# knagrecha/saturn

Measured on AMD Instinct MI355X. Metric: samples_per_s, higher is better.
Workload: dtype bf16; 1 GPU; model=gptj-6b, global_batch=16, seq_len=512, parallelism=dp1, optimizer=fused_sgd

## Files before the change

saturn_amd/ops/csrc/attention.hip:

```cpp

#include <torch/extension.h>
#include <ATen/hip/HIPContext.h>

#include <atomic>

#include "common.h"
#include "ops.h"

namespace samd {

typedef __attribute__((ext_vector_type(8))) short bf16x8;
typedef __attribute__((ext_vector_type(4))) float f32x4;

constexpr int QBLK = 64;
constexpr int KBLK = 32;
constexpr int WROWS = 16;

struct TStr {
  long sb, sh, st;
};
static TStr str_of(const at::Tensor& t) {
  return TStr{t.stride(0), t.stride(1), t.stride(2)};
}

// ... 130 lines not shown
#pragma unroll
      for (int c = 0; c < CHUNKS; ++c) {
        const int idx = (c * 256 + threadIdx.x) * 8;
        const int row = idx / D, col = idx % D;
        stg_k[c] = *reinterpret_cast<const bf16x8*>(
            Kh + (long)(kv0 + KBLK + row) * ks.st + col);
        stg_v[c] = *reinterpret_cast<const bf16x8*>(
            Vh + (long)(kv0 + KBLK + row) * vs.st + col);
      }
    }
    __syncthreads();

    f32x4 acc0 = {0.f, 0.f, 0.f, 0.f};
    f32x4 acc1 = {0.f, 0.f, 0.f, 0.f};
#pragma unroll
    for (int ds = 0; ds < D / 32; ++ds) {
      bf16x8 bk0 = *reinterpret_cast<const bf16x8*>(&lds.k[r][ds * 32 + qg * 8]);
      bf16x8 bk1 =
          *reinterpret_cast<const bf16x8*>(&lds.k[16 + r][ds * 32 + qg * 8]);
      acc0 = __builtin_amdgcn_mfma_f32_16x16x32_bf16(frag_q[ds], bk0, acc0, 0, 0, 0);
      acc1 = __builtin_amdgcn_mfma_f32_16x16x32_bf16(frag_q[ds], bk1, acc1, 0, 0, 0);
    }
#pragma unroll
    for (int reg = 0; reg < 4; ++reg) {
      const int row = qg * 4 + reg;
      const int qrow = q0 + row;
      float s0 = acc0[reg] * scale;
      float s1 = acc1[reg] * scale;
      if (causal) {
        if (kv0 + r > qrow) s0 = -INFINITY;
        if (kv0 + 16 + r > qrow) s1 = -INFINITY;
      }
      if (kv0 + r >= kv_len) s0 = -INFINITY;
      if (kv0 + 16 + r >= kv_len) s1 = -INFINITY;
      if constexpr (LO) {
        if (kv0 + r < lo_r[reg]) s0 = -INFINITY;
        if (kv0 + 16 + r < lo_r[reg]) s1 = -INFINITY;
      }
      float tm = fmaxf(s0, s1);
#pragma unroll
      for (int off = 1; off < 16; off <<= 1)
        tm = fmaxf(tm, __shfl_xor(tm, off, 64));
      const float m_new = fmaxf(m_reg[reg], tm);
      const float al =
          (m_reg[reg] == -INFINITY) ? 0.f : __expf(m_reg[reg] - m_new);
      const float p0 = (s0 == -INFINITY) ? 0.f : __expf(s0 - m_new);
      const float p1 = (s1 == -INFINITY) ? 0.f : __expf(s1 - m_new);
      float ps = p0 + p1;
#pragma unroll
      for (int off = 1; off < 16; off <<= 1)
        ps += __shfl_xor(ps, off, 64);
      l_reg[reg] = l_reg[reg] * al + ps;
      m_reg[reg] = m_new;
      lds.p[wid][row][r] = f2us(p0);
      lds.p[wid][row][16 + r] = f2us(p1);
#pragma unroll
      for (int dt = 0; dt < D / 16; ++dt) otile[dt][reg] *= al;
    }

    bf16x8 frag_p = *reinterpret_cast<const bf16x8*>(&lds.p[wid][r][qg * 8]);
#pragma unroll
    for (int dt = 0; dt < D / 16; ++dt) {
      bf16x8 bv = tr16_bfrag<D + 8>(&lds.v[qg * 8][dt * 16], lane);
      otile[dt] = __builtin_amdgcn_mfma_f32_16x16x32_bf16(frag_p, bv, otile[dt], 0, 0, 0);
    }
  }

  unsigned short* Oh = O + b * os.sb + h * os.sh;
#pragma unroll
  for (int reg = 0; reg < 4; ++reg) {
    int row = qg * 4 + reg;
    float linv = 1.f / l_reg[reg];
#pragma unroll
    for (int dt = 0; dt < D / 16; ++dt)
      Oh[(long)(q0 + row) * os.st + dt * 16 + r] =
          f2us(otile[dt][reg] * linv);
  }
  if (r == 0 && LSE != nullptr) {
#pragma unroll
    for (int reg = 0; reg < 4; ++reg)
      LSE[bh * (long)T + q0 + qg * 4 + reg] =
          m_reg[reg] + __logf(l_reg[reg]);
  }
}



typedef __attribute__((ext_vector_type(16))) float f32x16;

template <int D>
struct AttnV2Lds {
  unsigned short k[KBLK][D + 8];
  unsigned short v[KBLK][D + 8];
};

template <int D, bool LO>
__launch_bounds__(256, 2)
__global__ void attn_fwd_v2_kernel(const unsigned short* __restrict__ Q,
                                   const unsigned short* __restrict__ K,
                                   const unsigned short* __restrict__ V,
                                   unsigned short* __restrict__ O,
                                   float* __restrict__ LSE, int T,
                                   int n_heads, int n_kv, float scale,
                                   int causal, int kv_len, TStr qs,
                                   TStr ks, TStr vs,
                                   TStr os, const int* __restrict__ KVLO,
                                   long lo_sb) {
  extern __shared__ __attribute__((aligned(16))) char smem[];
  AttnV2Lds<D>& lds = *reinterpret_cast<AttnV2Lds<D>*>(smem);

  const int lane = threadIdx.x & 63;
  const int wid = threadIdx.x >> 6;
  const int qr = lane & 31;
  const int hi = lane >> 5;
  const long bh = blockIdx.x;
  const long b = bh / n_heads, h = bh % n_heads;
  const long h_kv = h * n_kv / n_heads;
  const int q0_block = blockIdx.y * (4 * 32);
  const int q0 = q0_block + wid * 32;
  const unsigned short* Qh = Q + b * qs.sb + h * qs.sh;
  const unsigned short* Kh = K + b * ks.sb + h_kv * ks.sh;
  const unsigned short* Vh = V + b * vs.sb + h_kv * vs.sh;

  constexpr bool QREG = (D < 256);
  bf16x8 frag_q[QREG ? D / 16 : 1];
  if constexpr (QREG) {
#pragma unroll
    for (int ds = 0; ds < D / 16; ++ds)
      frag_q[ds] = *reinterpret_cast<const bf16x8*>(
          Qh + (long)(q0 + qr) * qs.st + ds * 16 + hi * 8);
  }

  f32x16 oacc[D / 32];
#pragma unroll
  for (int dv = 0; dv < D / 32; ++dv)
#pragma unroll
    for (int e = 0; e < 16; ++e) oacc[dv][e] = 0.f;

  float m_row = -INFINITY, l_row = 0.f;

  int kv_begin = 0, lo_row = 0;
  if constexpr (LO) {
    const int* lo_b = KVLO + b * lo_sb;
    kv_begin = (lo_b[q0_block] / KBLK) * KBLK;
    lo_row = lo_b[q0 + qr];
  }

  constexpr int CHUNKS = (KBLK * D) / (256 * 8);
  bf16x8 stg_k[CHUNKS], stg_v[CHUNKS];
#pragma unroll
  for (int c = 0; c < CHUNKS; ++c) {
    const int idx = (c * 256 + threadIdx.x) * 8;
    const int row = idx / D, col = idx % D;
    stg_k[c] = *reinterpret_cast<const bf16x8*>(
        Kh + (long)(kv_begin + row) * ks.st + col);
    stg_v[c] = *reinterpret_cast<const bf16x8*>(
        Vh + (long)(kv_begin + row) * vs.st + col);
  }

  const int kv_end = causal ? (q0_block + 4 * 32) : T;
  for (int kv0 = kv_begin; kv0 < kv_end; kv0 += KBLK) {
    __syncthreads();
#pragma unroll
    for (int c = 0; c < CHUNKS; ++c) {
      const int idx = (c * 256 + threadIdx.x) * 8;
      const int row = idx / D, col = idx % D;
      *reinterpret_cast<bf16x8*>(&lds.k[row][col]) = stg_k[c];
      *reinterpret_cast<bf16x8*>(&lds.v[row][col]) = stg_v[c];
    }
    if (kv0 + KBLK < kv_end) {
#pragma unroll
      for (int c = 0; c < CHUNKS; ++c) {
        const int idx = (c * 256 + threadIdx.x) * 8;
        const int row = idx / D, col = idx % D;
        stg_k[c] = *reinterpret_cast<const bf16x8*>(
            Kh + (long)(kv0 + KBLK + row) * ks.st + col);
        stg_v[c] = *reinterpret_cast<const bf16x8*>(
            Vh + (long)(kv0 + KBLK + row) * vs.st + col);
      }
    }
    __syncthreads();

    f32x16 st;
#pragma unroll
    for (int e = 0; e < 16; ++e) st[e] = 0.f;
#pragma unroll
    for (int ds = 0; ds < D / 16; ++ds) {
      bf16x8 ak = *reinterpret_cast<const bf16x8*>(
          &lds.k[qr][ds * 16 + hi * 8]);
      bf16x8 fq;
      if constexpr (QREG)
        fq = frag_q[ds];
      else
        fq = *reinterpret_cast<const bf16x8*>(
            Qh + (long)(q0 + qr) * qs.st + ds * 16 + hi * 8);
      st = __builtin_amdgcn_mfma_f32_32x32x16_bf16(ak, fq, st, 0, 0, 0);
    }

    const int q_glob = q0 + qr;
    float p[16];
    float tile_max = -INFINITY;
#pragma unroll
    for (int reg = 0; reg < 16; ++reg) {
      const int key_loc = (reg & 3) + 8 * (reg >> 2) + 4 * hi;
      float sv = st[reg] * scale;
      if ((causal && kv0 + key_loc > q_glob) || kv0 + key_loc >= kv_len)
        sv = -INFINITY;
      if constexpr (LO) {
        if (kv0 + key_loc < lo_row) sv = -INFINITY;
      }
      p[reg] = sv;
      tile_max = fmaxf(tile_max, sv);
    }
    tile_max = fmaxf(tile_max, __shfl_xor(tile_max, 32, 64));
    const float m_new = fmaxf(m_row, tile_max);
    const float alpha = (m_row == -INFINITY) ? 0.f : __expf(m_row - m_new);
    float psum = 0.f;
#pragma unroll
    for (int reg = 0; reg < 16; ++reg) {
      const float pv = (p[reg] == -INFINITY) ? 0.f : __expf(p[reg] - m_new);
      p[reg] = pv;
      psum += pv;
    }
    psum += __shfl_xor(psum, 32, 64);
    l_row = l_row * alpha + psum;
    m_row = m_new;

    unsigned pk[8];
#pragma unroll
    for (int i = 0; i < 8; ++i) {
      const unsigned lo = f2us(p[2 * i]);
      const unsigned hi2 = f2us(p[2 * i + 1]);
      pk[i] = lo | (hi2 << 16);
    }
    bf16x8 pa[2];
#pragma unroll
    for (int g = 0; g < 2; ++g) {
      auto r0 = __builtin_amdgcn_permlane32_swap(pk[4 * g + 0], pk[4 * g + 2],
                                                 false, false);
      auto r1 = __builtin_amdgcn_permlane32_swap(pk[4 * g + 1], pk[4 * g + 3],
                                                 false, false);
      unsigned w0 = r0[0], w1 = r1[0], w2 = r0[1], w3 = r1[1];
      pa[g][0] = (short)(w0 & 0xffff);
      pa[g][1] = (short)(w0 >> 16);
      pa[g][2] = (short)(w1 & 0xffff);
      pa[g][3] = (short)(w1 >> 16);
      pa[g][4] = (short)(w2 & 0xffff);
      pa[g][5] = (short)(w2 >> 16);
      pa[g][6] = (short)(w3 & 0xffff);
      pa[g][7] = (short)(w3 >> 16);
    }

#pragma unroll
    for (int reg = 0; reg < 16; ++reg) {
      const int row = (reg & 3) + 8 * (reg >> 2) + 4 * hi;
      const float al = __shfl(alpha, row, 64);
#pragma unroll
      for (int dv = 0; dv < D / 32; ++dv) oacc[dv][reg] *= al;
    }

#pragma unroll
    for (int dv = 0; dv < D / 32; ++dv) {
#pragma unroll
      for (int g = 0; g < 2; ++g) {
        const int src_row = g * 16 + ((lane >> 4) & 2) * 4 + ((lane >> 2) & 3);
        const int src_col = dv * 32 + ((lane >> 4) & 1) * 16 + 4 * (lane & 3);
        const unsigned a0 = lds_addr32(&lds.v[src_row][src_col]);
        const unsigned a1 = a0 + 4u * (D + 8) * 2u;
        bf16x4 v0, v1;
        asm volatile(
            "ds_read_b64_tr_b16 %0, %2\n\t"
            "ds_read_b64_tr_b16 %1, %3\n\t"
            "s_waitcnt lgkmcnt(0)"
            : "=&v"(v0), "=&v"(v1)
            : "v"(a0), "v"(a1)
            : "memory");
        bf16x8 bv = __builtin_shufflevector(v0, v1, 0, 1, 2, 3, 4, 5, 6, 7);
        oacc[dv] = __builtin_amdgcn_mfma_f32_32x32x16_bf16(pa[g], bv,
                                                           oacc[dv], 0, 0, 0);
      }
    }
  }

  unsigned short* Oh = O + b * os.sb + h * os.sh;
  const float linv_own = 1.f / l_row;
#pragma unroll
  for (int reg = 0; reg < 16; ++reg) {
    const int row = (reg & 3) + 8 * (reg >> 2) + 4 * hi;
    const float linv = __shfl(linv_own, row, 64);
#pragma unroll
    for (int dv = 0; dv < D / 32; ++dv)
      Oh[(long)(q0 + row) * os.st + dv * 32 + qr] = f2us(oacc[dv][reg] * linv);
  }
  if (hi == 0 && LSE != nullptr)
    LSE[bh * (long)T + q0 + qr] = m_row + __logf(l_row);
}


namespace bwd {
constexpr int KB = 64;
constexpr int QT = 32;
}

template <int D, bool HASV>
struct AttnBwdLds {
  unsigned short kt[bwd::KB][D + 8];
  unsigned short vt[HASV ? bwd::KB : 1][D + 8];
  unsigned short qt[bwd::QT][D + 8];
  unsigned short dot[bwd::QT][D + 8];
  unsigned short pt[4][16][bwd::QT + 8];
  unsigned short dst[bwd::KB][bwd::QT + 8];
  float lse_t[bwd::QT];
  float delta_t[bwd::QT];
};
template <int D, bool HASV>
struct AttnBwdLdsLo : AttnBwdLds<D, HASV> {
  int lo_t[bwd::QT];
};
template <int D, bool HASV, bool LO>
using AttnBwdLdsT = typename std::conditional<LO, AttnBwdLdsLo<D, HASV>,
                                              AttnBwdLds<D, HASV>>::type;


template <int D>
__global__ void attn_delta_kernel(const unsigned short* __restrict__ dO,
                                  const unsigned short* __restrict__ O,
                                  float* __restrict__ delta, int T,
                                  int n_heads, TStr dos, TStr os) {
  const int lane = threadIdx.x & 63;
  const int wid = threadIdx.x >> 6;
  const long bh = blockIdx.y;
  const long b = bh / n_heads, h = bh % n_heads;
  const unsigned short* dOh = dO + b * dos.sb + h * dos.sh;
  const unsigned short* Oh = O + b * os.sb + h * os.sh;
  constexpr int EPL = D / 64;
  for (int t = blockIdx.x * 4 + wid; t < T; t += gridDim.x * 4) {
    float acc = 0.f;
    if constexpr (EPL >= 4) {
#pragma unroll
      for (int c = 0; c < EPL / 4; ++c) {
        const int off = (lane * (EPL / 4) + c * 64) * 4;
        bf16x4 a = *reinterpret_cast<const bf16x4*>(dOh + (long)t * dos.st + off);
        bf16x4 o4 = *reinterpret_cast<const bf16x4*>(Oh + (long)t * os.st + off);
#pragma unroll
        for (int e = 0; e < 4; ++e)
          acc += us2f((unsigned short)a[e]) * us2f((unsigned short)o4[e]);
      }
    } else {
#pragma unroll
      for (int e = 0; e < EPL; ++e) {
        const int off = lane * EPL + e;
        acc += us2f(dOh[(long)t * dos.st + off]) *
               us2f(Oh[(long)t * os.st + off]);
      }
    }
    acc = wave_allsum(acc);
    if (lane == 0) delta[bh * (long)T + t] = acc;
  }
}

template <int D, bool TR16, bool VL2, bool LO>
__launch_bounds__(256, 2)
__global__ void attn_bwd_kernel(const unsigned short* __restrict__ dO,
                                const unsigned short* __restrict__ Q,
                                const unsigned short* __restrict__ K,
                                const unsigned short* __restrict__ V,
                                const float* __restrict__ LSE,
                                const float* __restrict__ DELTA,
                                unsigned short* __restrict__ dK,
                                unsigned short* __restrict__ dV,
                                float* __restrict__ dKf,
                                float* __restrict__ dVf, int T, int n_heads,
                                int n_kv, float scale, int causal,
                                int kv_len, TStr dos,
                                TStr qs, TStr ks, TStr vs,
                                TStr dks, TStr dvs,
                                const int* __restrict__ KVLO, long lo_sb) {
  using namespace bwd;
  extern __shared__ __attribute__((aligned(16))) char smem[];
  constexpr bool HASV = (D <= 128) && !VL2;
  AttnBwdLdsT<D, HASV, LO>& lds =
      *reinterpret_cast<AttnBwdLdsT<D, HASV, LO>*>(smem);

  const int lane = threadIdx.x & 63;
  const int wid = threadIdx.x >> 6;
  const int r = lane & 15;
  const int qg = lane >> 4;
  const int kv0 = blockIdx.y * KB;
  const long bh = blockIdx.x;
  const long b = bh / n_heads, h = bh % n_heads;
  const long h_kv = h * n_kv / n_heads;
  const unsigned short* Qh = Q + b * qs.sb + h * qs.sh;
  const unsigned short* Kh = K + b * ks.sb + h_kv * ks.sh;
  const unsigned short* Vh = V + b * vs.sb + h_kv * vs.sh;
  const unsigned short* dOh = dO + b * dos.sb + h * dos.sh;
  const float* lse_h = LSE + bh * (long)T;
  const float* del_h = DELTA + bh * (long)T;
  const int* lo_b = nullptr;
  if constexpr (LO) lo_b = KVLO + b * lo_sb;

  {
    constexpr int CHUNKS = (KB * D) / (256 * 8);
#pragma unroll
    for (int c = 0; c < CHUNKS; ++c) {
      int idx = (c * 256 + threadIdx.x) * 8;
      int row = idx / D, col = idx % D;
      *reinterpret_cast<bf16x8*>(&lds.kt[row][col]) =
          *reinterpret_cast<const bf16x8*>(
              Kh + (long)(kv0 + row) * ks.st + col);
      if constexpr (HASV)
        *reinterpret_cast<bf16x8*>(&lds.vt[row][col]) =
            *reinterpret_cast<const bf16x8*>(
                Vh + (long)(kv0 + row) * vs.st + col);
    }
  }

  f32x4 acc_dv[D / 16], acc_dk[D / 16];
#pragma unroll
  for (int dt = 0; dt < D / 16; ++dt) {
    acc_dv[dt] = {0.f, 0.f, 0.f, 0.f};
    acc_dk[dt] = {0.f, 0.f, 0.f, 0.f};
  }

  const int q_start = causal ? kv0 : 0;
  for (int q0 = q_start; q0 < T; q0 += QT) {
    if constexpr (LO) {
      if (lo_b[q0] > kv0 + KB - 1) break;
    }
    __syncthreads();
    {
      constexpr int CHUNKS = (QT * D) / (256 * 8);
#pragma unroll
      for (int c = 0; c < CHUNKS; ++c) {
        int idx = (c * 256 + threadIdx.x) * 8;
        int row = idx / D, col = idx % D;
        *reinterpret_cast<bf16x8*>(&lds.qt[row][col]) =
            *reinterpret_cast<const bf16x8*>(
                Qh + (long)(q0 + row) * qs.st + col);
        *reinterpret_cast<bf16x8*>(&lds.dot[row][col]) =
            *reinterpret_cast<const bf16x8*>(
                dOh + (long)(q0 + row) * dos.st + col);
      }
      if (threadIdx.x < QT) {
        lds.lse_t[threadIdx.x] = lse_h[q0 + threadIdx.x];
        lds.delta_t[threadIdx.x] = del_h[q0 + threadIdx.x];
        if constexpr (LO) lds.lo_t[threadIdx.x] = lo_b[q0 + threadIdx.x];
      }
    }
    __syncthreads();

#pragma unroll
    for (int n = 0; n < 2; ++n) {
      f32x4 st = {0.f, 0.f, 0.f, 0.f};
      f32x4 dpt = {0.f, 0.f, 0.f, 0.f};
#pragma unroll
      for (int ds = 0; ds < D / 32; ++ds) {
        bf16x8 ak = *reinterpret_cast<const bf16x8*>(
            &lds.kt[wid * 16 + r][ds * 32 + qg * 8]);
        bf16x8 av;
        if constexpr (HASV)
          av = *reinterpret_cast<const bf16x8*>(
              &lds.vt[wid * 16 + r][ds * 32 + qg * 8]);
        else
          av = *reinterpret_cast<const bf16x8*>(
              Vh + (long)(kv0 + wid * 16 + r) * vs.st + ds * 32 + qg * 8);
        bf16x8 bq = *reinterpret_cast<const bf16x8*>(
            &lds.qt[n * 16 + r][ds * 32 + qg * 8]);
        bf16x8 bdo = *reinterpret_cast<const bf16x8*>(
            &lds.dot[n * 16 + r][ds * 32 + qg * 8]);
        st = __builtin_amdgcn_mfma_f32_16x16x32_bf16(ak, bq, st, 0, 0, 0);
        dpt = __builtin_amdgcn_mfma_f32_16x16x32_bf16(av, bdo, dpt, 0, 0, 0);
      }
#pragma unroll
      for (int reg = 0; reg < 4; ++reg) {
        const int key_loc = qg * 4 + reg;
        const int key_glob = kv0 + wid * 16 + key_loc;
        const int q_glob = q0 + n * 16 + r;
        float p = 0.f;
        bool seen = (!causal || q_glob >= key_glob) && key_glob < kv_len;
        if constexpr (LO) seen = seen && key_glob >= lds.lo_t[n * 16 + r];
        if (seen) {
          p = __expf(scale * st[reg] - lds.lse_t[n * 16 + r]);
        }
        const float dsv = p * (dpt[reg] - lds.delta_t[n * 16 + r]) * scale;
        lds.pt[wid][key_loc][n * 16 + r] = f2us(p);
        lds.dst[wid * 16 + key_loc][n * 16 + r] = f2us(dsv);
      }
    }

    {
      bf16x8 ap = *reinterpret_cast<const bf16x8*>(&lds.pt[wid][r][qg * 8]);
      bf16x8 adst =
          *reinterpret_cast<const bf16x8*>(&lds.dst[wid * 16 + r][qg * 8]);
#pragma unroll
      for (int dt = 0; dt < D / 16; ++dt) {
        bf16x8 bdo, bq;
        if constexpr (TR16) {
          tr16_bfrag2<D + 8, D + 8>(&lds.dot[qg * 8][dt * 16],
                                    &lds.qt[qg * 8][dt * 16], lane, bdo, bq);
        } else {
#pragma unroll
          for (int j = 0; j < 8; ++j) {
            bdo[j] = (short)lds.dot[qg * 8 + j][dt * 16 + r];
            bq[j] = (short)lds.qt[qg * 8 + j][dt * 16 + r];
          }
        }
        acc_dv[dt] =
            __builtin_amdgcn_mfma_f32_16x16x32_bf16(ap, bdo, acc_dv[dt], 0, 0, 0);
        acc_dk[dt] =
            __builtin_amdgcn_mfma_f32_16x16x32_bf16(adst, bq, acc_dk[dt], 0, 0, 0);
      }
    }

    __syncthreads();
  }

  if (n_kv != n_heads) {
    float* dKh = dKf + b * dks.sb + h_kv * dks.sh;
    float* dVh = dVf + b * dvs.sb + h_kv * dvs.sh;
#pragma unroll
    for (int reg = 0; reg < 4; ++reg) {
      const int key_glob = kv0 + wid * 16 + qg * 4 + reg;
#pragma unroll
      for (int dt = 0; dt < D / 16; ++dt) {
        atomicAdd(&dKh[(long)key_glob * dks.st + dt * 16 + r],
                  acc_dk[dt][reg]);
        atomicAdd(&dVh[(long)key_glob * dvs.st + dt * 16 + r],
                  acc_dv[dt][reg]);
      }
    }
  } else {
    unsigned short* dKh = dK + b * dks.sb + h * dks.sh;
    unsigned short* dVh = dV + b * dvs.sb + h * dvs.sh;
#pragma unroll
    for (int reg = 0; reg < 4; ++reg) {
      const int key_glob = kv0 + wid * 16 + qg * 4 + reg;
#pragma unroll
      for (int dt = 0; dt < D / 16; ++dt) {
        dKh[(long)key_glob * dks.st + dt * 16 + r] = f2us(acc_dk[dt][reg]);
        dVh[(long)key_glob * dvs.st + dt * 16 + r] = f2us(acc_dv[dt][reg]);
      }
    }
  }
}

namespace dq {
constexpr int QB = 64;
constexpr int KT = 32;
}

template <int D, bool GKV>
struct AttnDqLds {
  unsigned short qt[GKV ? 1 : dq::QB][D + 8];
  unsigned short dot[GKV ? 1 : dq::QB][D + 8];
  unsigned short kt[dq::KT][D + 8];
  unsigned short vt[GKV ? 1 : dq::KT][D + 8];
  float lse_t[dq::QB];
  float delta_t[dq::QB];
};

template <int D, bool TR16, bool GKV, bool LO>
__launch_bounds__(256, GKV ? 3 : (D <= 128 ? 2 : 1))
__global__ void attn_dq_kernel(const unsigned short* __restrict__ dO,
                               const unsigned short* __restrict__ Q,
                               const unsigned short* __restrict__ K,
                               const unsigned short* __restrict__ V,
                               const float* __restrict__ LSE,
                               const float* __restrict__ DELTA,
                               unsigned short* __restrict__ dQ16, int T,
                               int n_heads, int n_kv, float scale, int causal,
                               int kv_len, TStr dos, TStr qs, TStr ks,
                               TStr vs, TStr dqs,
                               const int* __restrict__ KVLO, long lo_sb) {
  using namespace dq;
  extern __shared__ __attribute__((aligned(16))) char smem[];
  AttnDqLds<D, GKV>& lds = *reinterpret_cast<AttnDqLds<D, GKV>*>(smem);

  const int lane = threadIdx.x & 63;
  const int wid = threadIdx.x >> 6;
  const int r = lane & 15;
  const int qg = lane >> 4;
  const int q0 = blockIdx.y * QB;
  const long bh = blockIdx.x;
  const long b = bh / n_heads, h = bh % n_heads;
  const long h_kv = h * n_kv / n_heads;
  const unsigned short* Qh = Q + b * qs.sb + h * qs.sh;
  const unsigned short* Kh = K + b * ks.sb + h_kv * ks.sh;
  const unsigned short* Vh = V + b * vs.sb + h_kv * vs.sh;
  const unsigned short* dOh = dO + b * dos.sb + h * dos.sh;
  const float* lse_h = LSE + bh * (long)T;
  const float* del_h = DELTA + bh * (long)T;

  {
    if constexpr (!GKV) {
      constexpr int CHUNKS = (QB * D) / (256 * 8);
#pragma unroll
      for (int c = 0; c < CHUNKS; ++c) {
        int idx = (c * 256 + threadIdx.x) * 8;
        int row = idx / D, col = idx % D;
        *reinterpret_cast<bf16x8*>(&lds.qt[row][col]) =
            *reinterpret_cast<const bf16x8*>(Qh + (long)(q0 + row) * qs.st + col);
        *reinterpret_cast<bf16x8*>(&lds.dot[row][col]) =
            *reinterpret_cast<const bf16x8*>(
                dOh + (long)(q0 + row) * dos.st + col);
      }
    }
    if (threadIdx.x < QB) {
      lds.lse_t[threadIdx.x] = lse_h[q0 + threadIdx.x];
      lds.delta_t[threadIdx.x] = del_h[q0 + threadIdx.x];
    }
  }

  f32x4 acc[D / 16];
#pragma unroll
  for (int dt = 0; dt < D / 16; ++dt) acc[dt] = {0.f, 0.f, 0.f, 0.f};

  const int k_end = causal ? (q0 + QB < T ? q0 + QB : T) : T;
  int k_begin = 0, lo_q = 0;
  if constexpr (LO) {
    const int* lo_b = KVLO + b * lo_sb;
    k_begin = (lo_b[q0] / KT) * KT;
    lo_q = lo_b[q0 + wid * 16 + r];
  }
  for (int k0 = k_begin; k0 < k_end; k0 += KT) {
    __syncthreads();
    {
      constexpr int CHUNKS = (KT * D) / (256 * 8);
#pragma unroll
      for (int c = 0; c < CHUNKS; ++c) {
        int idx = (c * 256 + threadIdx.x) * 8;
        int row = idx / D, col = idx % D;
        *reinterpret_cast<bf16x8*>(&lds.kt[row][col]) =
            *reinterpret_cast<const bf16x8*>(
                Kh + (long)(k0 + row) * ks.st + col);
        if constexpr (!GKV)
          *reinterpret_cast<bf16x8*>(&lds.vt[row][col]) =
              *reinterpret_cast<const bf16x8*>(
                  Vh + (long)(k0 + row) * vs.st + col);
      }
    }
    __syncthreads();

    if (causal && k0 > q0 + wid * 16 + 15) continue;

    float ds_sub[2][4];
#pragma unroll
    for (int n = 0; n < 2; ++n) {
      f32x4 st = {0.f, 0.f, 0.f, 0.f};
      f32x4 dpt = {0.f, 0.f, 0.f, 0.f};
#pragma unroll
      for (int ds_ = 0; ds_ < D / 32; ++ds_) {
        bf16x8 ak = *reinterpret_cast<const bf16x8*>(
            &lds.kt[n * 16 + r][ds_ * 32 + qg * 8]);
        bf16x8 av, bq, bdo;
        if constexpr (GKV) {
          av = *reinterpret_cast<const bf16x8*>(
              Vh + (long)(k0 + n * 16 + r) * vs.st + ds_ * 32 + qg * 8);
          bq = *reinterpret_cast<const bf16x8*>(
              Qh + (long)(q0 + wid * 16 + r) * qs.st + ds_ * 32 + qg * 8);
          bdo = *reinterpret_cast<const bf16x8*>(
              dOh + (long)(q0 + wid * 16 + r) * dos.st + ds_ * 32 + qg * 8);
        } else {
          av = *reinterpret_cast<const bf16x8*>(
              &lds.vt[n * 16 + r][ds_ * 32 + qg * 8]);
          bq = *reinterpret_cast<const bf16x8*>(
              &lds.qt[wid * 16 + r][ds_ * 32 + qg * 8]);
          bdo = *reinterpret_cast<const bf16x8*>(
              &lds.dot[wid * 16 + r][ds_ * 32 + qg * 8]);
        }
        st = __builtin_amdgcn_mfma_f32_16x16x32_bf16(ak, bq, st, 0, 0, 0);
        dpt = __builtin_amdgcn_mfma_f32_16x16x32_bf16(av, bdo, dpt, 0, 0, 0);
      }
      const int q_glob = q0 + wid * 16 + r;
      const float l_q = lds.lse_t[wid * 16 + r];
      const float d_q = lds.delta_t[wid * 16 + r];
#pragma unroll
      for (int reg = 0; reg < 4; ++reg) {
        const int key_glob = k0 + n * 16 + qg * 4 + reg;
        float p = 0.f;
        bool seen = (!causal || q_glob >= key_glob) && key_glob < kv_len;
        if constexpr (LO) seen = seen && key_glob >= lo_q;
        if (seen) p = __expf(scale * st[reg] - l_q);
        ds_sub[n][reg] = p * (dpt[reg] - d_q) * scale;
      }
    }

    unsigned pk[2][2];
#pragma unroll
    for (int n = 0; n < 2; ++n) {
      pk[n][0] = (unsigned)f2us(ds_sub[n][0]) |
                 ((unsigned)f2us(ds_sub[n][1]) << 16);
      pk[n][1] = (unsigned)f2us(ds_sub[n][2]) |
                 ((unsigned)f2us(ds_sub[n][3]) << 16);
    }
    const int a = (qg & 1) * 2;
    const int nsrc = qg >> 1;
    const int s0 = a * 16 + r;
    const int s1 = (a + 1) * 16 + r;
    unsigned rr[4][2];
#pragma unroll
    for (int nn = 0; nn < 2; ++nn) {
      rr[nn * 2 + 0][0] = (unsigned)__shfl((int)pk[nn][0], s0, 64);
      rr[nn * 2 + 0][1] = (unsigned)__shfl((int)pk[nn][1], s0, 64);
      rr[nn * 2 + 1][0] = (unsigned)__shfl((int)pk[nn][0], s1, 64);
      rr[nn * 2 + 1][1] = (unsigned)__shfl((int)pk[nn][1], s1, 64);
    }
    bf16x8 ads;
#pragma unroll
    for (int j = 0; j < 8; ++j) {
      const int src = (j >= 4) ? 1 : 0;
      const int reg = j & 3;
      const unsigned u = rr[nsrc * 2 + src][reg >> 1];
      ads[j] = (short)((reg & 1) ? (u >> 16) : (u & 0xffffu));
    }

#pragma unroll
    for (int dt = 0; dt < D / 16; ++dt) {
      bf16x8 bk;
      if constexpr (TR16) {
        bk = tr16_bfrag<D + 8>(&lds.kt[qg * 8][dt * 16], lane);
      } else {
#pragma unroll
        for (int j = 0; j < 8; ++j)
          bk[j] = (short)lds.kt[qg * 8 + j][dt * 16 + r];
      }
      acc[dt] = __builtin_amdgcn_mfma_f32_16x16x32_bf16(ads, bk, acc[dt], 0, 0, 0);
    }
  }

  unsigned short* dQh = dQ16 + b * dqs.sb + h * dqs.sh;
#pragma unroll
  for (int reg = 0; reg < 4; ++reg) {
    const int q_glob = q0 + wid * 16 + qg * 4 + reg;
#pragma unroll
    for (int dt = 0; dt < D / 16; ++dt)
      dQh[(long)q_glob * dqs.st + dt * 16 + r] = f2us(acc[dt][reg]);
  }
}


static bool env_is(const char* name, char c) {
  const char* e = getenv(name);
  return e && e[0] == c;
}
static bool sw_v2() {
  static const bool v = !env_is("SAMD_ATTN_V2", '0');
  return v;
}
static bool sw_tr16() {
  static const bool v = !env_is("SAMD_ATTN_BWD_TR16", '0');
  return v;
}
static bool sw_dq_gkv() {
  static const bool v = env_is("SAMD_ATTN_DQ_GKV", '1');
  return v;
}
static bool sw_vl2() {
  static const bool v = env_is("SAMD_ATTN_BWD_VL2", '1');
  return v;
}

struct AttnPlan {
  bool fwd_v2;
  bool tr16;
  bool vl2;
  bool gkv;
  bool lo;
};
static AttnPlan attn_plan(int T, int D, bool has_lo, bool bwd = true) {
  if (has_lo && bwd) {
    TORCH_CHECK(sw_tr16(), "attn_bwd: kv_lo is not built for "
                "SAMD_ATTN_BWD_TR16=0; unset the switch");
    TORCH_CHECK(!sw_vl2(), "attn_bwd: kv_lo is not built for "
                "SAMD_ATTN_BWD_VL2=1; unset the switch");
    TORCH_CHECK(!sw_dq_gkv(), "attn_bwd: kv_lo is not built for "
                "SAMD_ATTN_DQ_GKV=1; unset the switch");
  }
  return AttnPlan{sw_v2() && T % 128 == 0 && D <= 128, sw_tr16() && D <= 128,
                  sw_vl2() && D <= 128, sw_dq_gkv() && D > 128, has_lo};
}

template <class Fn>
struct Variant {
  Fn* kernel;
  int lds;
  int rows;
  std::atomic<bool>* lds_raised;
  const char* stem;
  int nargs, args[3];
  bool lo;
};
using FwdVariant = Variant<decltype(attn_fwd_kernel<64, false>)>;
using DeltaVariant = Variant<decltype(attn_delta_kernel<64>)>;
using BwdVariant = Variant<decltype(attn_bwd_kernel<64, false, false, false>)>;
using DqVariant = Variant<decltype(attn_dq_kernel<64, false, false, false>)>;

template <int D, bool LO>
static FwdVariant fwd_v1_of() {
  return {&attn_fwd_kernel<D, LO>, (int)sizeof(AttnLds<D>), QBLK, nullptr,
          "attn_fwd_kernel", 1, {D}, LO};
}
template <int D, bool LO>
static FwdVariant fwd_v2_of() {
  return {&attn_fwd_v2_kernel<D, LO>, (int)sizeof(AttnV2Lds<D>), 4 * 32,
          nullptr, "attn_fwd_v2_kernel", 1, {D}, LO};
}
template <int D>
static DeltaVariant delta_of() {
  return {&attn_delta_kernel<D>, 0, 4, nullptr, "attn_delta_kernel", 1, {D},
          false};
}
template <int D, bool TR16, bool VL2, bool LO>
static BwdVariant bwd_of() {
  static std::atomic<bool> raised{false};
  constexpr bool HASV = (D <= 128) && !VL2;
  return {&attn_bwd_kernel<D, TR16, VL2, LO>,
          (int)sizeof(AttnBwdLdsT<D, HASV, LO>), bwd::KB, &raised,
          "attn_bwd_kernel", 3, {D, TR16, VL2}, LO};
}
template <int D, bool TR16, bool GKV, bool LO>
static DqVariant dq_of() {
  static std::atomic<bool> raised{false};
  return {&attn_dq_kernel<D, TR16, GKV, LO>, (int)sizeof(AttnDqLds<D, GKV>),
          dq::QB, &raised, "attn_dq_kernel", 3, {D, TR16, GKV}, LO};
}

template <class F>
static auto with_d(int D, F f) {
  if (D == 64) return f(std::integral_constant<int, 64>{});
  if (D == 128) return f(std::integral_constant<int, 128>{});
  return f(std::integral_constant<int, 256>{});
}

static FwdVariant fwd_variant(const AttnPlan& p, int D) {
  return with_d(D, [&](auto d) -> FwdVariant {
    constexpr int DD = decltype(d)::value;
    if constexpr (DD <= 128) {
      if (p.fwd_v2) return p.lo ? fwd_v2_of<DD, true>() : fwd_v2_of<DD, false>();
    }
    return p.lo ? fwd_v1_of<DD, true>() : fwd_v1_of<DD, false>();
  });
}
static DeltaVariant delta_variant(int D) {
  return with_d(D, [](auto d) { return delta_of<decltype(d)::value>(); });
}
static BwdVariant bwd_variant(const AttnPlan& p, int D) {
  return with_d(D, [&](auto d) -> BwdVariant {
    constexpr int DD = decltype(d)::value;
    if (p.lo) return bwd_of<DD, (DD <= 128), false, true>();
    if constexpr (DD <= 128) {
      if (p.tr16)
        return p.vl2 ? bwd_of<DD, true, true, false>()
                     : bwd_of<DD, true, false, false>();
      if (p.vl2) return bwd_of<DD, false, true, false>();
    }
    return bwd_of<DD, false, false, false>();
  });
}
static DqVariant dq_variant(const AttnPlan& p, int D) {
  return with_d(D, [&](auto d) -> DqVariant {
    constexpr int DD = decltype(d)::value;
    if (p.lo) return dq_of<DD, (DD <= 128), false, true>();
    if constexpr (DD <= 128) {
      if (p.tr16) return dq_of<DD, true, false, false>();
    } else {
      if (p.gkv) return dq_of<DD, false, true, false>();
    }
    return dq_of<DD, false, false, false>();
  });
}

template <class Fn>
static std::string name_of(const Variant<Fn>& v) {
  std::string s = std::string(v.stem) + "<" + std::to_string(v.args[0]);
  for (int i = 1; i < v.nargs; ++i) s += "," + std::to_string(v.args[i]);
  return s + (v.lo ? ",1>" : ">");
}

std::string attn_dispatch(int64_t T, int64_t D, bool has_lo) {
  TORCH_CHECK(T > 0 && T % QBLK == 0, "attn_dispatch: T must be a multiple of 64");
  TORCH_CHECK(D == 64 || D == 128 || D == 256, "attn_dispatch: D in {64,128,256}");
  const int d = (int)D;
  const AttnPlan p = attn_plan((int)T, d, has_lo);
  return name_of(fwd_variant(p, d)) + " " + name_of(delta_variant(d)) + " " +
         name_of(bwd_variant(p, d)) + " " + name_of(dq_variant(p, d));
}

template <class Fn, class... Args>
static void launch(const Variant<Fn>& v, dim3 grid, hipStream_t stream,
                   Args... args) {
  if (v.lds_raised && !v.lds_raised->load(std::memory_order_relaxed)) {
    SAMD_CHECK_HIP(hipFuncSetAttribute(
        reinterpret_cast<const void*>(v.kernel),
        hipFuncAttributeMaxDynamicSharedMemorySize, v.lds));
    v.lds_raised->store(true, std::memory_order_relaxed);
  }
  hipLaunchKernelGGL(v.kernel, grid, dim3(256), v.lds, stream, args...);
  SAMD_CHECK_HIP(hipGetLastError());
}

static const unsigned short* bf16_in(const at::Tensor& t) {
  return reinterpret_cast<const unsigned short*>(t.data_ptr());
}
static unsigned short* bf16_out(const at::Tensor& t) {
  return reinterpret_cast<unsigned short*>(t.data_ptr());
}

struct LoArg {
  const int* ptr;
  long sb;
};
static LoArg lo_arg(const c10::optional<at::Tensor>& kv_lo,
                    const at::Tensor& q, bool causal, const char* who) {
  if (!kv_lo.has_value()) return LoArg{nullptr, 0};
  const at::Tensor& lo = *kv_lo;
  const int64_t B = q.size(0), T = q.size(2);
  TORCH_CHECK(causal, who, ": kv_lo requires causal=True");
  TORCH_CHECK(lo.scalar_type() == at::kInt, who, ": kv_lo must be int32");
  TORCH_CHECK(lo.is_cuda() && lo.device() == q.device(), who,
              ": kv_lo must be on q's device");
  TORCH_CHECK((lo.dim() == 1 && lo.size(0) == T) ||
                  (lo.dim() == 2 && lo.size(0) == B && lo.size(1) == T),
              who, ": kv_lo must have shape [T] or [B, T] (padded T)");
  TORCH_CHECK(lo.is_contiguous(), who, ": kv_lo must be contiguous");
  return LoArg{lo.data_ptr<int>(), lo.dim() == 2 ? (long)T : 0L};
}

struct AttnDims {
  int B, H, Hkv, T, D;
};
static bool bf16_on(const at::Tensor& t, const at::Tensor& q) {
  return t.scalar_type() == at::kBFloat16 && t.device() == q.device();
}
static AttnDims check_qkv(const at::Tensor& q, const at::Tensor& k,
                          const at::Tensor& v, int64_t& kv_len,
                          const char* who) {
  TORCH_CHECK(q.is_cuda() && q.scalar_type() == at::kBFloat16, who,
              ": bf16 only");
  TORCH_CHECK(q.dim() == 4 && k.dim() == 4 && v.dim() == 4, who,
              ": [B, H, T, D]");
  TORCH_CHECK(q.stride(3) == 1 && k.stride(3) == 1 && v.stride(3) == 1, who,
              ": innermost dim must be dense");
  const int B = (int)q.size(0), H = (int)q.size(1), T = (int)q.size(2),
            D = (int)q.size(3);
  const int Hkv = (int)k.size(1);
  TORCH_CHECK(Hkv > 0 && H % Hkv == 0, who,
              ": q heads must be a multiple of kv heads");
  TORCH_CHECK(k.size(2) == T, who, ": q/k length mismatch");
  TORCH_CHECK(T % QBLK == 0, who, ": T must be a multiple of 64");
  if (kv_len <= 0) kv_len = T;
  TORCH_CHECK(kv_len <= T, who, ": kv_len exceeds padded T");
  TORCH_CHECK(D == 64 || D == 128 || D == 256, who, ": D in {64,128,256}");
  TORCH_CHECK((reinterpret_cast<uintptr_t>(q.data_ptr()) & 15) == 0 &&
              q.stride(2) % 8 == 0 && k.stride(2) % 8 == 0 &&
              v.stride(2) % 8 == 0, who, ": rows must be 16-B aligned");
  TORCH_CHECK(bf16_on(k, q), who, ": k must be bf16 on q's device");
  TORCH_CHECK(bf16_on(v, q), who, ": v must be bf16 on q's device");
  TORCH_CHECK(k.size(0) == B && k.size(3) == D, who,
              ": k must be [B, Hkv, T, D] with q's B, T and D");
  TORCH_CHECK(v.sizes() == k.sizes(), who, ": v must have k's sizes");
  return AttnDims{B, H, Hkv, T, D};
}

std::vector<at::Tensor> attn_fwd(at::Tensor q, at::Tensor k, at::Tensor v,
                                 bool causal, int64_t kv_len,
                                 c10::optional<at::Tensor> kv_lo) {
  const auto [B, H, Hkv, T, D] = check_qkv(q, k, v, kv_len, "attn_fwd");
  const LoArg lo = lo_arg(kv_lo, q, causal, "attn_fwd");

  auto o_phys = at::empty({B, T, H, D}, q.options());
  auto o = o_phys.permute({0, 2, 1, 3});
  auto lse = at::empty({B, H, T}, q.options().dtype(at::kFloat));
  const float scale = 1.f / sqrtf((float)D);

  const FwdVariant fv =
      fwd_variant(attn_plan(T, D, lo.ptr != nullptr, false), D);
  launch(fv, dim3(B * H, T / fv.rows), at::hip::getCurrentHIPStream().stream(),
         bf16_in(q), bf16_in(k), bf16_in(v), bf16_out(o),
         lse.data_ptr<float>(), T, H, Hkv, scale, causal ? 1 : 0, (int)kv_len,
         str_of(q), str_of(k), str_of(v), str_of(o), lo.ptr, lo.sb);
  return {o, lse};
}

std::vector<at::Tensor> attn_bwd(at::Tensor dout, at::Tensor q, at::Tensor k,
                                 at::Tensor v, at::Tensor o, at::Tensor lse,
                                 bool causal, int64_t kv_len,
                                 c10::optional<at::Tensor> kv_lo) {
  const auto [B, H, Hkv, T, D] = check_qkv(q, k, v, kv_len, "attn_bwd");
  TORCH_CHECK(dout.sizes() == q.sizes(), "attn_bwd: dout must have q's sizes");
  TORCH_CHECK(o.sizes() == q.sizes(), "attn_bwd: o must have q's sizes");
  TORCH_CHECK(bf16_on(dout, q), "attn_bwd: dout must be bf16 on q's device");
  TORCH_CHECK(bf16_on(o, q), "attn_bwd: o must be bf16 on q's device");
  TORCH_CHECK(dout.stride(3) == 1, "attn_bwd: dout innermost dim must be dense");
  TORCH_CHECK(o.stride(3) == 1, "attn_bwd: o innermost dim must be dense");
  TORCH_CHECK(dout.stride(2) % 8 == 0, "attn_bwd: dout rows must be 16-B aligned");
  TORCH_CHECK(lse.scalar_type() == at::kFloat && lse.device() == q.device(),
              "attn_bwd: lse must be fp32 on q's device");
  TORCH_CHECK(lse.dim() == 3 && lse.size(0) == B && lse.size(1) == H &&
                  lse.size(2) == T && lse.is_contiguous(),
              "attn_bwd: lse must be a contiguous [B, H, T] tensor");
  const LoArg lo = lo_arg(kv_lo, q, causal, "attn_bwd");
  const AttnPlan plan = attn_plan(T, D, lo.ptr != nullptr);

  auto delta = at::empty({B, H, T}, q.options().dtype(at::kFloat));
  auto dq = at::empty({B, T, H, D}, q.options()).permute({0, 2, 1, 3});
  const bool gqa = Hkv != H;
  auto dk = at::empty({B, T, Hkv, D}, k.options()).permute({0, 2, 1, 3});
  auto dv = at::empty({B, T, Hkv, D}, v.options()).permute({0, 2, 1, 3});
  at::Tensor dk_f32, dv_f32;
  if (gqa) {
    dk_f32 = at::zeros({B, T, Hkv, D}, q.options().dtype(at::kFloat))
                 .permute({0, 2, 1, 3});
    dv_f32 = at::zeros({B, T, Hkv, D}, q.options().dtype(at::kFloat))
                 .permute({0, 2, 1, 3});
  }
  hipStream_t stream = at::hip::getCurrentHIPStream().stream();
  const float scale = 1.f / sqrtf((float)D);
  const int c = causal ? 1 : 0, kvl = (int)kv_len;

  launch(delta_variant(D), dim3(std::min((T + 3) / 4, 2048), B * H), stream,
         bf16_in(dout), bf16_in(o), delta.data_ptr<float>(), T, H,
         str_of(dout), str_of(o));
  const DqVariant qv = dq_variant(plan, D);
  launch(qv, dim3(B * H, T / qv.rows), stream, bf16_in(dout), bf16_in(q),
         bf16_in(k), bf16_in(v), lse.data_ptr<float>(),
         delta.data_ptr<float>(), bf16_out(dq), T, H, Hkv, scale, c, kvl,
         str_of(dout), str_of(q), str_of(k), str_of(v), str_of(dq), lo.ptr,
         lo.sb);
  const BwdVariant bv = bwd_variant(plan, D);
  launch(bv, dim3(B * H, T / bv.rows), stream, bf16_in(dout), bf16_in(q),
         bf16_in(k), bf16_in(v), lse.data_ptr<float>(),
         delta.data_ptr<float>(), bf16_out(dk), bf16_out(dv),
         gqa ? dk_f32.data_ptr<float>() : nullptr,
         gqa ? dv_f32.data_ptr<float>() : nullptr, T, H, Hkv, scale, c, kvl,
         str_of(dout), str_of(q), str_of(k), str_of(v),
         gqa ? str_of(dk_f32) : str_of(dk), gqa ? str_of(dv_f32) : str_of(dv),
         lo.ptr, lo.sb);
  if (gqa) return {dq, dk_f32.to(at::kBFloat16), dv_f32.to(at::kBFloat16)};
  return {dq, dk, dv};
}

}
```

Baseline: 65.90 samples/s.

## Register-prefetch next Q/dO and K/V tiles in attention backward, vectorize dK/dV/dQ stores

Adds a PIPE variant of the attention backward and dQ kernels, on by default for D of 128 and 256. Each loop iteration loads the next Q/dO (or K/V) tile into registers while the current tile is computed, then writes it to LDS, dropping one __syncthreads per iteration. dK, dV and dQ outputs are now staged through LDS and written as 128-bit rows instead of scattered 16-bit stores. The cost is more registers per thread, which may lower occupancy, plus more template complexity and a new row-stride limit check.

```diff
diff --git a/saturn_amd/ops/csrc/attention.hip b/saturn_amd/ops/csrc/attention.hip
--- a/saturn_amd/ops/csrc/attention.hip
+++ b/saturn_amd/ops/csrc/attention.hip
@@ -456,6 +456,39 @@
 constexpr int QT = 32;
 }
 
+template <int D>
+__device__ __forceinline__ void store_tile_b128(
+    unsigned short (*tile)[D + 8], const f32x4 (&acc)[D / 16],
+    unsigned short* __restrict__ dst, long st, int lane) {
+  const int r = lane & 15, qg = lane >> 4;
+  const bool odd = (r & 1) != 0;
+  const int row0 = qg * 4 + (odd ? 2 : 0);
+#pragma unroll
+  for (int dt = 0; dt < D / 16; ++dt) {
+    const unsigned p01 = (unsigned)f2us(acc[dt][0]) |
+                         ((unsigned)f2us(acc[dt][1]) << 16);
+    const unsigned p23 = (unsigned)f2us(acc[dt][2]) |
+                         ((unsigned)f2us(acc[dt][3]) << 16);
+    const unsigned mine = odd ? p23 : p01;
+    const unsigned got =
+        (unsigned)__shfl_xor((int)(odd ? p01 : p23), 1, 64);
+    const unsigned lo = odd ? got : mine;
+    const unsigned hi = odd ? mine : got;
+    *reinterpret_cast<unsigned*>(&tile[row0][dt * 16 + (r & ~1)]) =
+        (lo & 0xffffu) | (hi << 16);
+    *reinterpret_cast<unsigned*>(&tile[row0 + 1][dt * 16 + (r & ~1)]) =
+        (lo >> 16) | (hi & 0xffff0000u);
+  }
+  __builtin_amdgcn_wave_barrier();
+#pragma unroll
+  for (int i = 0; i < D / 32; ++i) {
+    const int vi = i * 64 + lane;
+    const int row = vi / (D / 8), col = (vi % (D / 8)) * 8;
+    *reinterpret_cast<bf16x8*>(dst + (long)row * st + col) =
+        *reinterpret_cast<const bf16x8*>(&tile[row][col]);
+  }
+}
+
 template <int D, bool HASV>
 struct AttnBwdLds {
   unsigned short kt[bwd::KB][D + 8];
@@ -474,6 +507,11 @@
 template <int D, bool HASV, bool LO>
 using AttnBwdLdsT = typename std::conditional<LO, AttnBwdLdsLo<D, HASV>,
                                               AttnBwdLds<D, HASV>>::type;
+static_assert(sizeof(AttnBwdLdsLo<256, false>) ==
+                  sizeof(AttnBwdLds<256, false>) + sizeof(int) * bwd::QT &&
+              sizeof(AttnBwdLdsLo<64, true>) ==
+                  sizeof(AttnBwdLds<64, true>) + sizeof(int) * bwd::QT,
+              "lo_t must follow delta_t directly");
 
 
 template <int D>
@@ -513,7 +551,7 @@
   }
 }
 
-template <int D, bool TR16, bool VL2, bool LO>
+template <int D, bool TR16, bool VL2, bool LO, bool PIPE>
 __launch_bounds__(256, 2)
 __global__ void attn_bwd_kernel(const unsigned short* __restrict__ dO,
                                 const unsigned short* __restrict__ Q,
@@ -537,7 +575,8 @@
       *reinterpret_cast<AttnBwdLdsT<D, HASV, LO>*>(smem);
 
   const int lane = threadIdx.x & 63;
-  const int wid = threadIdx.x >> 6;
+  const int wid = PIPE ? __builtin_amdgcn_readfirstlane(threadIdx.x >> 6)
+                       : (int)(threadIdx.x >> 6);
   const int r = lane & 15;
   const int qg = lane >> 4;
   const int kv0 = blockIdx.y * KB;
@@ -577,31 +616,85 @@
   }
 
   const int q_start = causal ? kv0 : 0;
-  for (int q0 = q_start; q0 < T; q0 += QT) {
-    if constexpr (LO) {
-      if (lo_b[q0] > kv0 + KB - 1) break;
-    }
-    __syncthreads();
-    {
-      constexpr int CHUNKS = (QT * D) / (256 * 8);
-#pragma unroll
-      for (int c = 0; c < CHUNKS; ++c) {
-        int idx = (c * 256 + threadIdx.x) * 8;
-        int row = idx / D, col = idx % D;
-        *reinterpret_cast<bf16x8*>(&lds.qt[row][col]) =
-            *reinterpret_cast<const bf16x8*>(
-                Qh + (long)(q0 + row) * qs.st + col);
-        *reinterpret_cast<bf16x8*>(&lds.dot[row][col]) =
-            *reinterpret_cast<const bf16x8*>(
-                dOh + (long)(q0 + row) * dos.st + col);
-      }
-      if (threadIdx.x < QT) {
-        lds.lse_t[threadIdx.x] = lse_h[q0 + threadIdx.x];
-        lds.delta_t[threadIdx.x] = del_h[q0 + threadIdx.x];
-        if constexpr (LO) lds.lo_t[threadIdx.x] = lo_b[q0 + threadIdx.x];
-      }
-    }
-    __syncthreads();
+  constexpr int QCH = (QT * D) / (256 * 8);
+  bf16x8 stg_q[PIPE ? QCH : 1], stg_do[PIPE ? QCH : 1];
+  unsigned stg_row = 0;
+  constexpr int RPC = (256 * 8) / D;
+  const unsigned boff_q =
+      2u * (unsigned)((threadIdx.x * 8 / D) * qs.st + (threadIdx.x * 8) % D);
+  const unsigned boff_do =
+      2u * (unsigned)((threadIdx.x * 8 / D) * dos.st + (threadIdx.x * 8) % D);
+  auto stage_load = [&](int qn) {
+#pragma unroll
+    for (int c = 0; c < QCH; ++c) {
+      stg_q[c] = *reinterpret_cast<const bf16x8*>(
+          reinterpret_cast<const char*>(Qh + (long)(qn + c * RPC) * qs.st) +
+          boff_q);
+      stg_do[c] = *reinterpret_cast<const bf16x8*>(
+          reinterpret_cast<const char*>(dOh + (long)(qn + c * RPC) * dos.st) +
+          boff_do);
+    }
+    const int i = threadIdx.x & (QT - 1);
+    if (threadIdx.x < QT) {
+      stg_row = __float_as_uint(lse_h[qn + i]);
+    } else if (threadIdx.x < 2 * QT) {
+      stg_row = __float_as_uint(del_h[qn + i]);
+    } else if (threadIdx.x < 3 * QT) {
+      if constexpr (LO) stg_row = (unsigned)lo_b[qn + i];
+    }
+  };
+  bool have = q_start < T;
+  if constexpr (PIPE) {
+    if constexpr (LO) have = have && !(lo_b[q_start] > kv0 + KB - 1);
+    if (have) stage_load(q_start);
+  }
+  for (int q0 = q_start; PIPE ? have : (q0 < T); q0 += QT) {
+    bool next = false;
+    if constexpr (PIPE) {
+      next = q0 + QT < T;
+      if constexpr (LO) next = next && !(lo_b[q0 + QT] > kv0 + KB - 1);
+      __syncthreads();
+#pragma unroll
+      for (int c = 0; c < QCH; ++c) {
+        const int idx = (c * 256 + threadIdx.x) * 8;
+        const int row = idx / D, col = idx % D;
+        *reinterpret_cast<bf16x8*>(&lds.qt[row][col]) = stg_q[c];
+        *reinterpret_cast<bf16x8*>(&lds.dot[row][col]) = stg_do[c];
+      }
+      if (threadIdx.x < (LO ? 3 : 2) * QT)
+        reinterpret_cast<unsigned*>(
+            smem + sizeof(lds) - (LO ? 3 : 2) * QT * sizeof(float))
+            [threadIdx.x] = stg_row;
+      if constexpr (HASV) {
+        if (next) stage_load(q0 + QT);
+      }
+      __syncthreads();
+    } else {
+      if constexpr (LO) {
+        if (lo_b[q0] > kv0 + KB - 1) break;
+      }
+      __syncthreads();
+      {
+        constexpr int CHUNKS = (QT * D) / (256 * 8);
+#pragma unroll
+        for (int c = 0; c < CHUNKS; ++c) {
+          int idx = (c * 256 + threadIdx.x) * 8;
+          int row = idx / D, col = idx % D;
+          *reinterpret_cast<bf16x8*>(&lds.qt[row][col]) =
+              *reinterpret_cast<const bf16x8*>(
+                  Qh + (long)(q0 + row) * qs.st + col);
+          *reinterpret_cast<bf16x8*>(&lds.dot[row][col]) =
+              *reinterpret_cast<const bf16x8*>(
+                  dOh + (long)(q0 + row) * dos.st + col);
+        }
+        if (threadIdx.x < QT) {
+          lds.lse_t[threadIdx.x] = lse_h[q0 + threadIdx.x];
+          lds.delta_t[threadIdx.x] = del_h[q0 + threadIdx.x];
+          if constexpr (LO) lds.lo_t[threadIdx.x] = lo_b[q0 + threadIdx.x];
+        }
+      }
+      __syncthreads();
+    }
 
 #pragma unroll
     for (int n = 0; n < 2; ++n) {
@@ -642,6 +735,10 @@
       }
     }
 
+    if constexpr (PIPE && !HASV) {
+      if (next) stage_load(q0 + QT);
+    }
+
     {
       bf16x8 ap = *reinterpret_cast<const bf16x8*>(&lds.pt[wid][r][qg * 8]);
       bf16x8 adst =
@@ -666,7 +763,10 @@
       }
     }
 
-    __syncthreads();
+    if constexpr (PIPE)
+      have = next;
+    else
+      __syncthreads();
   }
 
   if (n_kv != n_heads) {
@@ -683,6 +783,15 @@
                   acc_dv[dt][reg]);
       }
     }
+  } else if constexpr (PIPE) {
+    unsigned short* dKh = dK + b * dks.sb + h * dks.sh;
+    unsigned short* dVh = dV + b * dvs.sb + h * dvs.sh;
+    __syncthreads();
+    store_tile_b128<D>(&lds.kt[wid * 16], acc_dk,
+                       dKh + (long)(kv0 + wid * 16) * dks.st, dks.st, lane);
+    __builtin_amdgcn_wave_barrier();
+    store_tile_b128<D>(&lds.kt[wid * 16], acc_dv,
+                       dVh + (long)(kv0 + wid * 16) * dvs.st, dvs.st, lane);
   } else {
     unsigned short* dKh = dK + b * dks.sb + h * dks.sh;
     unsigned short* dVh = dV + b * dvs.sb + h * dvs.sh;
@@ -713,7 +822,7 @@
   float delta_t[dq::QB];
 };
 
-template <int D, bool TR16, bool GKV, bool LO>
+template <int D, bool TR16, bool GKV, bool LO, bool PIPE>
 __launch_bounds__(256, GKV ? 3 : (D <= 128 ? 2 : 1))
 __global__ void attn_dq_kernel(const unsigned short* __restrict__ dO,
                                const unsigned short* __restrict__ Q,
@@ -776,9 +885,40 @@
     k_begin = (lo_b[q0] / KT) * KT;
     lo_q = lo_b[q0 + wid * 16 + r];
   }
+  static_assert(!(PIPE && GKV), "the GKV probe keeps the single-buffered loop");
+  constexpr int KCH = (KT * D) / (256 * 8);
+  bf16x8 stg_k[PIPE ? KCH : 1], stg_v[PIPE ? KCH : 1];
+  constexpr int RPC = (256 * 8) / D;
+  const unsigned boff_k =
+      2u * (unsigned)((threadIdx.x * 8 / D) * ks.st + (threadIdx.x * 8) % D);
+  const unsigned boff_v =
+      2u * (unsigned)((threadIdx.x * 8 / D) * vs.st + (threadIdx.x * 8) % D);
+  auto stage_load = [&](int kn) {
+#pragma unroll
+    for (int c = 0; c < KCH; ++c) {
+      stg_k[c] = *reinterpret_cast<const bf16x8*>(
+          reinterpret_cast<const char*>(Kh + (long)(kn + c * RPC) * ks.st) +
+          boff_k);
+      stg_v[c] = *reinterpret_cast<const bf16x8*>(
+          reinterpret_cast<const char*>(Vh + (long)(kn + c * RPC) * vs.st) +
+          boff_v);
+    }
+  };
+  if constexpr (PIPE) {
+    if (k_begin < k_end) stage_load(k_begin);
+  }
   for (int k0 = k_begin; k0 < k_end; k0 += KT) {
     __syncthreads();
-    {
+    if constexpr (PIPE) {
+#pragma unroll
+      for (int c = 0; c < KCH; ++c) {
+        const int idx = (c * 256 + threadIdx.x) * 8;
+        const int row = idx / D, col = idx % D;
+        *reinterpret_cast<bf16x8*>(&lds.kt[row][col]) = stg_k[c];
+        *reinterpret_cast<bf16x8*>(&lds.vt[row][col]) = stg_v[c];
+      }
+      if (k0 + KT < k_end) stage_load(k0 + KT);
+    } else {
       constexpr int CHUNKS = (KT * D) / (256 * 8);
 #pragma unroll
       for (int c = 0; c < CHUNKS; ++c) {
@@ -883,12 +1023,18 @@
   }
 
   unsigned short* dQh = dQ16 + b * dqs.sb + h * dqs.sh;
-#pragma unroll
-  for (int reg = 0; reg < 4; ++reg) {
-    const int q_glob = q0 + wid * 16 + qg * 4 + reg;
-#pragma unroll
-    for (int dt = 0; dt < D / 16; ++dt)
-      dQh[(long)q_glob * dqs.st + dt * 16 + r] = f2us(acc[dt][reg]);
+  if constexpr (PIPE) {
+    __syncthreads();
+    store_tile_b128<D>(&lds.qt[wid * 16], acc,
+                       dQh + (long)(q0 + wid * 16) * dqs.st, dqs.st, lane);
+  } else {
+#pragma unroll
+    for (int reg = 0; reg < 4; ++reg) {
+      const int q_glob = q0 + wid * 16 + qg * 4 + reg;
+#pragma unroll
+      for (int dt = 0; dt < D / 16; ++dt)
+        dQh[(long)q_glob * dqs.st + dt * 16 + r] = f2us(acc[dt][reg]);
+    }
   }
 }
 
@@ -913,6 +1059,12 @@
   static const bool v = env_is("SAMD_ATTN_BWD_VL2", '1');
   return v;
 }
+
+static bool sw_pipe() {
+  static const bool v = !env_is("SAMD_ATTN_BWD_PIPE", '0');
+  return v;
+}
+constexpr bool pipe_built(int D) { return D == 256 || D == 128; }
 
 struct AttnPlan {
   bool fwd_v2;
@@ -920,6 +1072,7 @@
   bool vl2;
   bool gkv;
   bool lo;
+  bool pipe;
 };
 static AttnPlan attn_plan(int T, int D, bool has_lo, bool bwd = true) {
   if (has_lo && bwd) {
@@ -931,7 +1084,8 @@
                 "SAMD_ATTN_DQ_GKV=1; unset the switch");
   }
   return AttnPlan{sw_v2() && T % 128 == 0 && D <= 128, sw_tr16() && D <= 128,
-                  sw_vl2() && D <= 128, sw_dq_gkv() && D > 128, has_lo};
+                  sw_vl2() && D <= 128, sw_dq_gkv() && D > 128, has_lo,
+                  sw_pipe()};
 }
 
 template <class Fn>
@@ -943,11 +1097,14 @@
   const char* stem;
   int nargs, args[3];
   bool lo;
+  bool nopipe = false;
 };
 using FwdVariant = Variant<decltype(attn_fwd_kernel<64, false>)>;
 using DeltaVariant = Variant<decltype(attn_delta_kernel<64>)>;
-using BwdVariant = Variant<decltype(attn_bwd_kernel<64, false, false, false>)>;
-using DqVariant = Variant<decltype(attn_dq_kernel<64, false, false, false>)>;
+using BwdVariant =
+    Variant<decltype(attn_bwd_kernel<64, false, false, false, false>)>;
+using DqVariant =
+    Variant<decltype(attn_dq_kernel<64, false, false, false, false>)>;
 
 template <int D, bool LO>
 static FwdVariant fwd_v1_of() {
@@ -964,19 +1121,40 @@
   return {&attn_delta_kernel<D>, 0, 4, nullptr, "attn_delta_kernel", 1, {D},
           false};
 }
-template <int D, bool TR16, bool VL2, bool LO>
+constexpr bool pipe_form(int D, bool tr16, bool probe) {
+  return pipe_built(D) && tr16 == (D <= 128) && !probe;
+}
+template <int D, bool TR16, bool VL2, bool LO, bool PIPE>
 static BwdVariant bwd_of() {
+  static_assert(!PIPE || pipe_form(D, TR16, VL2), "no pipelined form");
   static std::atomic<bool> raised{false};
   constexpr bool HASV = (D <= 128) && !VL2;
-  return {&attn_bwd_kernel<D, TR16, VL2, LO>,
+  return {&attn_bwd_kernel<D, TR16, VL2, LO, PIPE>,
           (int)sizeof(AttnBwdLdsT<D, HASV, LO>), bwd::KB, &raised,
-          "attn_bwd_kernel", 3, {D, TR16, VL2}, LO};
-}
-template <int D, bool TR16, bool GKV, bool LO>
+          "attn_bwd_kernel", 3, {D, TR16, VL2}, LO,
+          !PIPE && pipe_form(D, TR16, VL2)};
+}
+template <int D, bool TR16, bool GKV, bool LO, bool PIPE>
 static DqVariant dq_of() {
+  static_assert(!PIPE || pipe_form(D, TR16, GKV), "no pipelined form");
   static std::atomic<bool> raised{false};
-  return {&attn_dq_kernel<D, TR16, GKV, LO>, (int)sizeof(AttnDqLds<D, GKV>),
-          dq::QB, &raised, "attn_dq_kernel", 3, {D, TR16, GKV}, LO};
+  return {&attn_dq_kernel<D, TR16, GKV, LO, PIPE>,
+          (int)sizeof(AttnDqLds<D, GKV>), dq::QB, &raised, "attn_dq_kernel", 3,
+          {D, TR16, GKV}, LO, !PIPE && pipe_form(D, TR16, GKV)};
+}
+template <int D, bool LO>
+static BwdVariant bwd_default_of(bool pipe) {
+  if constexpr (pipe_built(D)) {
+    if (pipe) return bwd_of<D, (D <= 128), false, LO, true>();
+  }
+  return bwd_of<D, (D <= 128), false, LO, false>();
+}
+template <int D, bool LO>
+static DqVariant dq_default_of(bool pipe) {
+  if constexpr (pipe_built(D)) {
+    if (pipe) return dq_of<D, (D <= 128), false, LO, true>();
+  }
+  return dq_of<D, (D <= 128), false, LO, false>();
 }
 
 template <class F>
@@ -1001,26 +1179,28 @@
 static BwdVariant bwd_variant(const AttnPlan& p, int D) {
   return with_d(D, [&](auto d) -> BwdVariant {
     constexpr int DD = decltype(d)::value;
-    if (p.lo) return bwd_of<DD, (DD <= 128), false, true>();
+    if (p.lo) return bwd_default_of<DD, true>(p.pipe);
     if constexpr (DD <= 128) {
       if (p.tr16)
-        return p.vl2 ? bwd_of<DD, true, true, false>()
-                     : bwd_of<DD, true, false, false>();
-      if (p.vl2) return bwd_of<DD, false, true, false>();
-    }
-    return bwd_of<DD, false, false, false>();
+        return p.vl2 ? bwd_of<DD, true, true, false, false>()
+                     : bwd_default_of<DD, false>(p.pipe);
+      if (p.vl2) return bwd_of<DD, false, true, false, false>();
+      return bwd_of<DD, false, false, false, false>();
+    }
+    return bwd_default_of<DD, false>(p.pipe);
   });
 }
 static DqVariant dq_variant(const AttnPlan& p, int D) {
   return with_d(D, [&](auto d) -> DqVariant {
     constexpr int DD = decltype(d)::value;
-    if (p.lo) return dq_of<DD, (DD <= 128), false, true>();
+    if (p.lo) return dq_default_of<DD, true>(p.pipe);
     if constexpr (DD <= 128) {
-      if (p.tr16) return dq_of<DD, true, false, false>();
+      if (p.tr16) return dq_default_of<DD, false>(p.pipe);
+      return dq_of<DD, false, false, false, false>();
     } else {
-      if (p.gkv) return dq_of<DD, false, true, false>();
-    }
-    return dq_of<DD, false, false, false>();
+      if (p.gkv) return dq_of<DD, false, true, false, false>();
+      return dq_default_of<DD, false>(p.pipe);
+    }
   });
 }
 
@@ -1028,7 +1208,7 @@
 static std::string name_of(const Variant<Fn>& v) {
   std::string s = std::string(v.stem) + "<" + std::to_string(v.args[0]);
   for (int i = 1; i < v.nargs; ++i) s += "," + std::to_string(v.args[i]);
-  return s + (v.lo ? ",1>" : ">");
+  return s + (v.lo ? ",1>" : ">") + (v.nopipe ? ".nopipe" : "");
 }
 
 std::string attn_dispatch(int64_t T, int64_t D, bool has_lo) {
@@ -1148,6 +1328,9 @@
   TORCH_CHECK(dout.stride(3) == 1, "attn_bwd: dout innermost dim must be dense");
   TORCH_CHECK(o.stride(3) == 1, "attn_bwd: o innermost dim must be dense");
   TORCH_CHECK(dout.stride(2) % 8 == 0, "attn_bwd: dout rows must be 16-B aligned");
+  for (const at::Tensor* t : {&dout, &q, &k, &v})
+    TORCH_CHECK(t->stride(2) >= 0 && t->stride(2) < (1L << 27),
+                "attn_bwd: row strides must be below 2^27 elements");
   TORCH_CHECK(lse.scalar_type() == at::kFloat && lse.device() == q.device(),
               "attn_bwd: lse must be fp32 on q's device");
   TORCH_CHECK(lse.dim() == 3 && lse.size(0) == B && lse.size(1) == H &&
```

After: 65.34 samples/s. About the same (-0.9%).
